# AE-HYU/monte_carlo_localization

Measured on AMD Instinct MI355X. Metric: MCL updates/sec (particle*beam/s), higher is better.
Workload: dtype f64; 1 GPU; 4194304 particles/GPU x 1081 beams, Spielberg_map (2000x2000 @ 0.05796), initial cloud N((0.0, 0.0, 0.0),(0.5 m,0.5 m,0.4 rad)) (tracking regime), action (0.05, 0.0, 0.01), stock sensor/motion params, multinomial resampling, Philox seed 42; the timed updates follow 5 warm-up updates (the particle set has resampled to motion-noise width); particles_total=4194304, beams=1081, parallelism=single GPU

## Files before the change

### include/mcl_hip_engine.h

```cpp
#ifndef MCL_HIP_ENGINE_H
#define MCL_HIP_ENGINE_H

#include <stddef.h>
#include <stdint.h>

#ifdef __cplusplus
extern "C" {
#endif

#define MCL_ABI_VERSION 1

typedef struct mcl_engine mcl_engine_t;

typedef enum {
    MCL_OK = 0,
    MCL_ERR_INVALID_ARG = -1,
    MCL_ERR_NOT_READY = -2,
    MCL_ERR_HIP = -3,
    MCL_ERR_NO_DEVICE = -4,
    MCL_ERR_UNSUPPORTED = -5,
    MCL_ERR_PEER = -6,
    MCL_ERR_TIMEOUT = -7
} mcl_status;

// ... 320 lines not shown
int mcl_host_skip_field(const int8_t *data, uint32_t width, uint32_t height, uint8_t *out, size_t n);
int mcl_host_skip_field_dir(const int8_t *data, uint32_t width, uint32_t height, int32_t quadrant, uint8_t *out, size_t n);
#define MCL_WEDGES 16
int mcl_host_skip_field_wedge(const int8_t *data, uint32_t width, uint32_t height, int32_t wedge, uint8_t *out, size_t n);
int mcl_host_skip_field_wedge_tight(const int8_t *data, uint32_t width, uint32_t height, int32_t wedge, uint8_t *out, size_t n);
int mcl_host_wedge_tight_table(int32_t wedge, int32_t *values, uint8_t *reachable, size_t n);
int mcl_host_sweep_global_layout(uint32_t width, uint32_t height, int32_t max_range_px, int64_t out[6]);
int mcl_get_wedge_fields(mcl_engine_t *h, uint8_t *out, size_t n, int32_t dims[3]);
int mcl_get_ring_fields(mcl_engine_t *h, uint8_t *out, size_t n);
int mcl_get_sweep_table(mcl_engine_t *h, double *out, size_t n, int32_t dims[3]);
int mcl_host_sort_key(const int32_t bbox[7], const int32_t *tilemap, int32_t ntx_abs, uint32_t width, uint32_t height,
                      const double *px, const double *py, const double *theta, int64_t n, int64_t n_layout, int32_t fine, uint32_t *keys);
int mcl_get_sort_order(mcl_engine_t *h, uint32_t *keys, uint32_t *perm, size_t n, int32_t bbox[7], int32_t *tilemap, size_t n_tiles,
                       int64_t *n_out, int32_t *fine);
int mcl_get_sort_record_form(mcl_engine_t *h, int32_t *heading_form);

typedef enum {
    MCL_BUF_X = 0, MCL_BUF_Y = 1, MCL_BUF_THETA = 2,
    MCL_BUF_QWEIGHT = 3,
    MCL_BUF_LOGW = 4,
    MCL_BUF_SCALARS = 5
} mcl_buffer_id;
int mcl_device_ptr(mcl_engine_t *h, int32_t which, void **dev_ptr);
int mcl_export_state(mcl_engine_t *h, double *d_x, double *d_y, double *d_theta, uint64_t *d_q);
int mcl_get_scalars(mcl_engine_t *h, double out[8]);
int mcl_get_host_scalars(const mcl_engine_t *h, double out[8]);
int mcl_stage_propagate(mcl_engine_t *h, const double *d_px, const double *d_py, const double *d_pth,
                        const uint64_t *d_cdf, int64_t n_parents, uint64_t q_total,
                        int64_t child_first, int64_t n_children_total,
                        const double action[3], const float *obs, int32_t n_beams);
// ... 74 lines not shown
```

### monte_carlo_localization_amd/csrc/mcl_engine.hip

```cpp
#include "../../include/mcl_hip_engine.h"

#include <hip/hip_runtime.h>
#include <hip/hip_ext.h>
#include <rocprim/device/device_radix_sort.hpp>

#include <algorithm>
#include <chrono>
#include <cmath>
#include <cstdio>
#include <cstring>
#include <string>
#include <vector>

#include "mcl_engine_internal.h"
#include "mcl_kernels.h"
#include "mcl_host_math.h"
#include "mcl_lfield.h"
#include "mcl_mount.h"

static_assert(MCL_WEDGES == mcl::kWedges || MCL_KWEDGES != 16, "include/mcl_hip_engine.h and csrc/mcl_wedge.h disagree");

using namespace mcl_host;

namespace {
// ... 66 lines not shown
    if (h->last_sweep_global == 2) {
        if (h->h_result[15] >= mcl::kFarWindowedMin / 2) { h->hyb_backoff = h->hyb_backoff ? std::min(32, 2 * h->hyb_backoff) : 1; h->hyb_skip = h->hyb_backoff; }
        else h->hyb_backoff = 0;
    }
    if (h->hyb_skip > 0) { --h->hyb_skip; return false; }
    return true;
}

int sweep_play(const mcl_engine *h, bool hybrid)
{
    if (hybrid) return mcl::kSwSide - (mcl::kSwHybReach + 2) - 3;
    if (h->sweep_global) return 1 << 20;
    return mcl::kSwSide - (h->P + 2) - 3;
}

int unit_play(const mcl_engine *h, int mode, bool hybrid)
{
    return h->env.no_bucket_cuts ? -1 : (mode_sweep(mode) ? sweep_play(h, hybrid) : 0);
}

int64_t max_sweep_units(int64_t n) { return (n + mcl::kSwUnit - 1) / mcl::kSwUnit + mcl::kSwMaxCuts + 2; }

int launch_sweep_plan(mcl_engine *h, int64_t n, int nwg, int g, bool hybrid)
{
    const int ngroups = mcl::kWedges / g;
    MCL_TRY(h->d_items.reserve(h, (size_t)max_sweep_units(n) * ngroups));
    MCL_TRY(h->d_centres.reserve(h, (size_t)max_sweep_units(n)));
    MCL_TRY(h->d_nitems.reserve(h, 1));
    const int play = sweep_play(h, hybrid);
    hipExtLaunchKernelGGL(mcl::k_sweep_plan, dim3(1), dim3(1024), mcl::kPlanLds, h->stream, nullptr, h->ev[EV_K0], 0, h->d_unit_sums.p, h->d_nunits.p, ngroups, nwg,
                          (double)(play / 2 - 1), h->env.sw_guide > 0 ? h->env.sw_guide : (h->sweep_global ? 3 : 2), h->d_items.p, h->d_centres.p, h->d_nitems.p);
    HIPCHK(h, hipGetLastError());
    return MCL_OK;
// ... 225 lines not shown

void ray_prep(mcl_engine *h, const RayPlan &p, const mcl::RayArgs &a)
{
    const dim3 grid((unsigned)((a.n + 255) / 256));
    if (!p.lists) {
        if (p.mode == MCL_RAYS_SKIP && !p.constants_ready)
            hipLaunchKernelGGL(mcl::k_particle_prep, grid, dim3(256), 0, h->stream, a.x, a.y, a.th, a.n, h->ox, h->oy, h->res, h->d_pc, h->d_angle, h->B,
                               (short4 *)nullptr, mcl::PrepClear{});
        return;
    }
    mcl::PrepClear clr{};
    clr.logw_acc = h->d_logw_acc; clr.far_flags = reinterpret_cast<uint32_t *>(h->d_far.p);
    clr.fix_count = h->d_fix_count; clr.fix_words = p.nseg * 8; clr.fix_over = h->d_fix_over; clr.exact_count = h->d_result + 14;
    if (p.sweep) clr.far_count = h->d_result + 15;
    if (p.ordered && !p.stale_layout) clr.bbox = h->d_bbox;
    clr.bbox_play = unit_play(h, p.mode, p.hyb);
    if (p.ordered && p.constants_ready) {
        clr.logw_acc = nullptr; clr.far_flags = nullptr;
        const mcl::PrepClear &pc0 = p.clear_passed;
        const bool done = p.clear_folded && clr.fix_count == pc0.fix_count && clr.fix_words == pc0.fix_words &&
                          clr.fix_over == pc0.fix_over && clr.exact_count == pc0.exact_count && clr.far_count == pc0.far_count &&
                          clr.bbox == pc0.bbox && clr.bbox_play == pc0.bbox_play && !clr.hist && !pc0.hist;
        if (!done) hipLaunchKernelGGL(mcl::k_prep_small, dim3(1), dim3(256), 0, h->stream, clr);
        if (!h->capturing) { h->prep_cache = clr; h->prep_cache_valid = true; h->prep_cache_n = a.n; }
    } else {
        hipLaunchKernelGGL(mcl::k_particle_prep, grid, dim3(256), 0, h->stream, a.x, a.y, a.th, a.n, h->ox, h->oy, h->res, h->d_pc, h->d_angle, h->B,
                           p.ordered ? (short4 *)nullptr : h->d_qr, clr);
    }
}

void ray_kernel_march(mcl_engine *h, const RayPlan &p, const mcl::RayArgs &a)
// ... 15 lines not shown
        hipLaunchKernelGGL(mcl::k_hist_partials, dim3(nparts), dim3(256), 0, h->stream, h->d_hist, h->d_histpart, h->d_tile_used);
        hipLaunchKernelGGL(mcl::k_hist_final, dim3(nparts), dim3(256), 0, h->stream, h->d_hist, h->d_histpart, h->d_tile_used);
        hipLaunchKernelGGL(mcl::k_sort_scatter, dim3(nb256), dim3(256), 0, h->stream, h->d_pc, a.th, n, h->d_skey, h->d_srank,
                           h->d_hist, h->d_pcs, h->d_ths, h->d_perm);
        return MCL_OK;
    }
    MCL_TRY(h->d_skey2.reserve(h, (size_t)h->cap));
    MCL_TRY(h->d_sval2.reserve(h, (size_t)h->cap));
    const int fine = sort_fine(h), key_bits = mcl::kSortKeyLog2 + mcl::sort_fine_bits(fine);
    size_t tb = 0;
    HIPCHK(h, rocprim::radix_sort_pairs(nullptr, tb, h->d_skey.p, h->d_skey2.p, h->d_srank.p, h->d_sval2.p, (size_t)n, 0, key_bits, h->stream));
    MCL_TRY(h->d_sort_tmp.reserve(h, tb));
    if (!(p.stale_layout && p.keys_written))
        hipLaunchKernelGGL(mcl::k_sort_keys, dim3(nb256), dim3(256), 0, h->stream, h->d_pc, a.th, n, h->Wp, h->Hp, h->d_bbox, h->d_skey, h->d_srank,
                           h->d_tilemap, ntx_abs, fine);
    tb = h->d_sort_tmp.cap;
    HIPCHK(h, rocprim::radix_sort_pairs(h->d_sort_tmp.p, tb, h->d_skey.p, h->d_skey2.p, h->d_srank.p, h->d_sval2.p, (size_t)n, 0, key_bits, h->stream));
    hipLaunchKernelGGL(mcl::k_sort_gather, dim3(nb256), dim3(256), 0, h->stream, h->d_pc, a.th, n, h->d_sval2, h->d_pcs, h->d_ths, h->d_perm,
                       p.sweep ? h->d_skey2 : (const uint32_t *)nullptr, h->d_bbox, h->d_cut_start, h->d_cut_end, fine, p.heading_form ? 1 : 0);
    h->order_last = {h->d_bbox.p, h->d_tilemap.p, n, fine, p.heading_form};
    return MCL_OK;
}

int ray_units(mcl_engine *h, const RayPlan &p, mcl::RayArgs &a)
{
    const int64_t n = a.n;
    const int nparts = (int)(mcl::kSortKeySpace / mcl::kHistTile);
    if (p.sweep) {
        const size_t mu = (size_t)max_sweep_units(n);
        MCL_TRY(h->d_unit_sums.reserve(h, mu * 2));
        MCL_TRY(h->d_unit_begin.reserve(h, mu + 1));
        MCL_TRY(h->d_nunits.reserve(h, 1));
        hipLaunchKernelGGL(mcl::k_unit_table, dim3(1), dim3(1024), 0, h->stream, h->d_bbox, n, h->d_hist, h->d_histpart, h->d_tile_used,
                           p.radix ? h->d_cut_start : (uint32_t *)nullptr, h->d_cut_end, h->d_unit_begin, h->d_nunits, (int)mu);
        hipLaunchKernelGGL(mcl::k_unit_sums, dim3((unsigned)std::min<int64_t>(max_sweep_units(n), (n + mcl::kSwUnit - 1) / mcl::kSwUnit + 256)), dim3(256), 0, h->stream, h->d_pcs, h->d_unit_begin, h->d_nunits,
                           h->d_unit_sums, p.radix ? (uint32_t *)nullptr : h->d_hist, h->d_tile_used, nparts);
    } else {
        if (!p.radix) hipLaunchKernelGGL(mcl::k_hist_clear, dim3(nparts), dim3(256), 0, h->stream, h->d_hist, h->d_tile_used);
        MCL_TRY(h->d_slice_mean.reserve(h, (size_t)p.nsl));
        hipLaunchKernelGGL(mcl::k_slice_means, dim3((unsigned)p.nsl), dim3(256), 0, h->stream, h->d_pcs, n, (n + p.nsl - 1) / p.nsl, h->d_slice_mean);
    }
    a.pcs = h->d_pcs; a.ths = h->d_ths; a.perm = h->d_perm; a.slice_mean = h->d_slice_mean;
    a.distw = h->d_distw; a.distw_stride = (size_t)h->Hp * h->Wps;
    return MCL_OK;
}

int ray_sweep_items(mcl_engine *h, const RayPlan &p, mcl::RayArgs &a)
{
    if (!h->d_Ltd) return fail(h, MCL_ERR_HIP, "k_rays_sweep: table not allocated (internal)");
    if (!h->ltd_ready) build_ltd(h);
    MCL_TRY(launch_sweep_plan(h, a.n, p.nseg, p.sweep_g, p.hyb));
// ... 450 lines not shown
const char *mcl_last_error(const mcl_engine_t *h) { return h ? h->err.c_str() : g_create_error.c_str(); }

static EnvKnobs read_knobs()
{
    EnvKnobs k;
    if (const char *e = getenv("MCL_CELL_MIN")) k.cell_min = atoll(e);
    if (const char *e = getenv("MCL_CELL_SLICE")) k.cell_slice = atoll(e);
    if (const char *e = getenv("MCL_QSLICES_PER_CU")) k.qslices_per_cu = atoi(e);
    if (const char *e = getenv("MCL_QSIDE")) k.qside = atoi(e);
    if (const char *e = getenv("MCL_SWEEP_G")) k.sweep_g = atoi(e);
    if (const char *e = getenv("MCL_TINY_POLL")) k.tiny_poll = atoi(e);
    if (const char *e = getenv("MCL_NO_COMPACT")) k.no_compact = atoi(e);
    if (const char *e = getenv("MCL_SORT")) k.sort_radix = std::strcmp(e, "radix") == 0 ? 1 : (std::strcmp(e, "hist") == 0 ? 0 : -1);
    if (const char *e = getenv("MCL_SORT_FINE")) k.sort_fine = atoi(e);
    if (const char *e = getenv("MCL_SORT_FINE_SUB")) k.sort_fine_sub = atoi(e);
    if (const char *e = getenv("MCL_FIX_WG")) k.fix_wg = atoi(e);
    if (const char *e = getenv("MCL_FIX_DEAL")) k.fix_deal_seg = std::strcmp(e, "seg") == 0;
    if (const char *e = getenv("MCL_DEBUG_WG")) k.debug_wg = e;
    k.no_bucket_cuts = getenv("MCL_NO_BUCKET_CUTS") != nullptr;
    if (const char *e = getenv("MCL_SWEEP_GLOBAL")) k.sweep_global = atoi(e) != 0;
    if (const char *e = getenv("MCL_SWEEP_HYBRID")) k.sweep_hybrid = atoi(e);
    if (const char *e = getenv("MCL_SW_GUIDE")) k.sw_guide = atoi(e);
    if (const char *e = getenv("MCL_SW_SPLIT16")) k.sw_split16 = atoi(e) != 0;
    if (const char *e = getenv("MCL_SWEEP_PAIRS")) k.sweep_pairs = atoi(e) != 0 ? 1 : 0;
    k.no_obs_overlap = getenv("MCL_NO_OBS_OVERLAP") != nullptr;
    k.no_prep_fold = getenv("MCL_NO_PREP_FOLD") != nullptr;
    k.no_stale_layout = getenv("MCL_NO_STALE_LAYOUT") != nullptr;
    k.comm_no_pregather = getenv("MCL_COMM_NO_PREGATHER") != nullptr;
    k.comm_no_lists = getenv("MCL_COMM_NO_LISTS") != nullptr;
    return k;
// ... 658 lines not shown
}

static int layout_mark(mcl_engine *h, int64_t n)
{
    h->layout.wanted = false;
    if (!mode_orders(choose_ray_mode(h, n, false)) || h->env.no_stale_layout) return MCL_OK;
    HIPCHK(h, hipEventRecord(h->layout.ev_children, h->stream));
    h->layout.wanted = true;
    return MCL_OK;
}

static int next_layout_launch(mcl_engine *h, int64_t n)
{
    if (!h->layout.wanted) return MCL_OK;
    h->layout.wanted = false;
    const int play = unit_play(h, choose_ray_mode(h, n, false), sweep_hybrid(h));
    HIPCHK(h, hipStreamWaitEvent(h->stream2, h->layout.ev_children, 0));
    hipLaunchKernelGGL(mcl::k_bbox_init, dim3(1), dim3(64), 0, h->stream2, h->layout.d_bbox_nx, play);
    launch_layout(h, h->stream2, n, h->layout.d_bbox_nx, h->layout.d_tilemark_nx, h->layout.d_tilemap_nx);
    HIPCHK(h, hipGetLastError());
    HIPCHK(h, hipEventRecord(h->layout.ev_layout, h->stream2));
    h->layout.pending = true;
    return MCL_OK;
}

int mcl_host::layout_adopt(mcl_engine *h, int64_t n)
{
    if (!h->layout.pending) return MCL_OK;
    HIPCHK(h, hipEventSynchronize(h->layout.ev_layout));
    std::swap(h->d_bbox, h->layout.d_bbox_nx); std::swap(h->d_tilemap, h->layout.d_tilemap_nx);
    h->layout.valid = true; h->layout.n = n; h->layout.pending = false;
// ... 841 lines not shown
        HIPCHK(h, hipMemcpyAsync(tilemap, o.tilemap, n_tiles * sizeof(int32_t), hipMemcpyDeviceToHost, h->stream));
    }
    HIPCHK(h, hipStreamSynchronize(h->stream));
    return MCL_OK;
}

int mcl_get_sort_record_form(mcl_engine_t *h, int32_t *heading_form)
{
    if (!h || !heading_form) return MCL_ERR_INVALID_ARG;
    const OrderLast &o = h->order_last;
    if (!o.bbox || o.n <= 0) return fail(h, MCL_ERR_NOT_READY, "the last ray stage did not order its particles through the radix sort");
    *heading_form = o.heading ? 1 : 0;
    return MCL_OK;
}

int mcl_get_ring_fields(mcl_engine_t *h, uint8_t *out, size_t n)
{
    if (!h || !out) return MCL_ERR_INVALID_ARG;
    if (!h->have_map || !h->d_distg) return fail(h, MCL_ERR_NOT_READY, "no map is set or the engine holds no ringed copies of the wedge fields");
    if (n != h->distg_stride * (size_t)mcl::kWedges) return fail(h, MCL_ERR_INVALID_ARG, "the ringed fields have the bytes of mcl_host_sweep_global_layout's allocation");
    HIPCHK(h, hipSetDevice(h->cfg.device));
    HIPCHK(h, hipMemcpyAsync(out, h->d_distg, n, hipMemcpyDeviceToHost, h->stream));
    HIPCHK(h, hipStreamSynchronize(h->stream));
    return MCL_OK;
}

int mcl_get_sweep_table(mcl_engine_t *h, double *out, size_t n, int32_t dims[3])
{
    if (!h) return MCL_ERR_INVALID_ARG;
    if (!h->have_map || h->B <= 0 || !h->d_Ltd || !h->ltd_ready)
// ... 632 lines not shown
```

### monte_carlo_localization_amd/csrc/mcl_engine_internal.h

```cpp
#pragma once
#include "../../include/mcl_hip_engine.h"

#include <hip/hip_runtime.h>
#include <hip/hip_ext.h>

#include <cstdint>
#include <string>
#include <vector>

#include "mcl_types.h"
#include "mcl_host_math.h"
#include "mcl_buffers.h"

enum { EV_START = 0, EV_RESAMPLE, EV_QUERY, EV_RAYS, EV_SENSOR, EV_K0, EV_K1, EV_COUNT };


constexpr unsigned long long kExactCap = 1ull << 16;
constexpr int kResultWords = 18;
constexpr int kResultStage = 40;
constexpr int kResultStamp = 32;

struct mcl_comm;
void comm_free(struct mcl_comm *c);
void comm_forget(struct mcl_comm *c);
// ... 18 lines not shown
    bool rays_bound = false;
    bool query_skipped = false;
};
struct NextLayout {
    bool wanted = false, pending = false, valid = false; int64_t n = 0;
    hipEvent_t ev_children = nullptr, ev_layout = nullptr;
    DevBuf<int> d_bbox_nx, d_tilemap_nx, d_tilemark_nx;
};
struct EnvKnobs {
    int64_t cell_min = 0, cell_slice = 0;
    int qslices_per_cu = 0, qside = 0, sweep_g = 0;
    int tiny_poll = 1, no_compact = 0;
    int sort_radix = -1;
    int sort_fine = -1;
    int sort_fine_sub = -1;
    int fix_wg = 0;
    bool fix_deal_seg = false;
    std::string debug_wg;
    bool no_bucket_cuts = false;
    bool sweep_global = false;
    int sweep_hybrid = 1;
    int sw_guide = 0;
    int sw_split16 = -1;
    int sweep_pairs = -1;
    bool no_obs_overlap = false;
    bool no_prep_fold = false;
    bool no_stale_layout = false;
    bool comm_no_pregather = false;
    bool comm_no_lists = false;
};
// ... 79 lines not shown
    unsigned long long list_epoch = 0;
    DevBuf<uint64_t> d_gcdf, d_gtop;
    DevBuf<double4> d_pcs;
    DevBuf<double> d_ths;
    DevBuf<uint32_t> d_perm, d_skey, d_srank;
    DevBuf<uint32_t> d_skey2, d_sval2;
    DevBuf<uint8_t> d_sort_tmp;
    DevBuf<uint32_t> d_tile_used;
    DevBuf<uint32_t> d_hist, d_histpart;
    DevBuf<int> d_bbox;
    OrderLast order_last;
    DevBuf<uint32_t> d_cut_start, d_cut_end;
    DevBuf<int> d_tilemap, d_tilemark;
    DevBuf<double2> d_slice_mean;
    DevBuf<double4> d_unit_sums;
    DevBuf<uint32_t> d_unit_begin;
    DevBuf<int> d_nunits;
    DevBuf<double4> d_pc;
    DevBuf<short4> d_qr;
    DevBuf<uint8_t> d_steps;
    DevBuf<unsigned long long> d_fix_list, d_fix_count;
    unsigned long long *d_fix_over = nullptr;
    DevBuf<unsigned long long> d_exact_list;
    unsigned long long fix_cap = 0; int fix_segments = 0;
    DevBuf<uint8_t> d_far;
    DevBuf<uint32_t> d_far_list;
    DevBuf<uint32_t> d_far_sorted, d_far_cnt;
    DevBuf<int4> d_items;
    DevBuf<int4> d_centres;
    DevBuf<int> d_nitems;
// ... 157 lines not shown
```

### monte_carlo_localization_amd/csrc/mcl_kernels.h

```cpp
#pragma once
#include "mcl_types.h"
#include <type_traits>
#include "mcl_ray_core.h"
#include "mcl_device_math.h"
#include "mcl_wedge.h"
#include "mcl_motion.h"
#include "mcl_sort_key.h"

namespace mcl {

constexpr int kRedBlocks = 1024;
constexpr int kRedThreads = 256;
__device__ __forceinline__ void final_sums_of(const double *__restrict__ part, int nb, double *__restrict__ scalars, double (*sm)[7]);


__device__ __forceinline__ uint64_t wave_incl_scan_u64(uint64_t v, int lane)
{
#pragma unroll
    for (int o = 1; o < 64; o <<= 1) {
        uint64_t t = (uint64_t)__shfl_up((long long)v, o, 64);
        if (lane >= o) v += t;
    }
    return v;
}
// ... 1311 lines not shown
__global__ __launch_bounds__(256) void k_sort_keys(const double4 *__restrict__ pc, const double *__restrict__ th, int64_t n, int Wp, int Hp,
                                                  const int *__restrict__ bbox, uint32_t *__restrict__ key_out, uint32_t *__restrict__ val_out,
                                                  const int *__restrict__ tilemap, int ntx_abs, int fine)
{
    const int64_t i = (int64_t)blockIdx.x * blockDim.x + threadIdx.x;
    if (i >= n) return;
    const double4 c = pc[i];
    key_out[i] = sort_key(bbox, tilemap, ntx_abs, cell_of(c.z * kSortSub, Wp * kSortSub - 1), cell_of(c.w * kSortSub, Hp * kSortSub - 1), th[i], n,
                          c.z * kSortSub - floor(c.z * kSortSub), c.w * kSortSub - floor(c.w * kSortSub), fine);
    val_out[i] = (uint32_t)i;
}
__global__ __launch_bounds__(256) void k_sort_gather(const double4 *__restrict__ pc, const double *__restrict__ th, int64_t n,
                                                    const uint32_t *__restrict__ order, double4 *__restrict__ pcs, double *__restrict__ ths,
                                                    uint32_t *__restrict__ perm, const uint32_t *__restrict__ sorted_keys = nullptr,
                                                    const int *__restrict__ bbox = nullptr, uint32_t *__restrict__ cut_start = nullptr,
                                                    uint32_t *__restrict__ cut_end = nullptr, int fine = 0, int heading_form = 0)
{
    const int64_t s = (int64_t)blockIdx.x * blockDim.x + threadIdx.x;
    if (s >= n) return;
    const uint32_t i = order[s];
    const double4 rec = pc[i];
    if (heading_form) { pcs[s] = particle_constants_of(rec); ths[s] = rec.x; }
    else { pcs[s] = rec; ths[s] = th[i]; }
    perm[s] = i;
    if (sorted_keys) {
        const SortLayout L = sort_layout(bbox, n, fine);
        if (L.cuts()) {
            const int sh = L.cut_shift();
            const uint32_t g = sorted_keys[s] >> sh;
            const uint32_t gp = s > 0 ? sorted_keys[s - 1] >> sh : 0xFFFFFFFFu;
            if (g != gp && g < (uint32_t)kSwMaxCuts) {
                cut_start[g] = (uint32_t)s + 1u;
                if (s > 0 && gp < (uint32_t)kSwMaxCuts) cut_end[gp] = (uint32_t)s;
            }
            if (s == n - 1 && g < (uint32_t)kSwMaxCuts) cut_end[g] = (uint32_t)n;
        }
    }
}

__global__ __launch_bounds__(256) void k_hist_clear(uint32_t *__restrict__ hist, uint32_t *__restrict__ tile_used)
{
    if (!tile_used[blockIdx.x]) return;
    const uint4 z = make_uint4(0u, 0u, 0u, 0u);
    for (int x = 0; x < kSortXcds; ++x) {
        uint4 *p = reinterpret_cast<uint4 *>(hist + (size_t)x * kSortKeySpace + (size_t)blockIdx.x * kHistTile) + threadIdx.x * 4;
#pragma unroll
        for (int k = 0; k < 4; ++k) p[k] = z;
    }
    __syncthreads();
    if (threadIdx.x == 0) tile_used[blockIdx.x] = 0u;
}
// ... 708 lines not shown
```

### monte_carlo_localization_amd/csrc/mcl_rays_sweep.h

```cpp
#pragma once

namespace mcl {

constexpr int kSwUnder = 127;
constexpr int kSwUnit = 1024;
constexpr int kSwFx = 32;
constexpr int kSwSide = 256;
#ifndef MCL_SW_PITCH
#define MCL_SW_PITCH 260
#endif
constexpr int kSwPitch = MCL_SW_PITCH;
static_assert(kSwPitch >= kSwSide && (kSwPitch % 4) == 0, "window rows are written as dwords");
constexpr int kSwWinBytes = kSwSide * kSwPitch;
#ifndef MCL_SW_HYB_PLAY
#define MCL_SW_HYB_PLAY 40
#endif
constexpr int kSwHybPlay = MCL_SW_HYB_PLAY;
constexpr int kSwHybReach = kSwSide - (kSwHybPlay + 3) - 2;
#if MCL_KWEDGES == 8
__device__ constexpr double kSwHybInvDx[2] = {1.0, 1.414213562373095};
__device__ constexpr double kSwHybInvDy[2] = {1.4142135623730951, 1.0};
#elif MCL_KWEDGES == 16
__device__ constexpr double kSwHybInvDx[4] = {1.0, 1.082392200292394, 1.414213562373095, 2.6131259297527527};
__device__ constexpr double kSwHybInvDy[4] = {2.613125929752753, 1.4142135623730951, 1.082392200292394, 1.0};
// ... 111 lines not shown
        }
        if (threadIdx.x == 1023) carry_sh = at + nu;
        __syncthreads();
        if (threadIdx.x == 0) nbig_sh = 0u;
        __syncthreads();
    }
    if (threadIdx.x == 0) {
        int M = (int)carry_sh;
        if (M > max_units) M = max_units;
        ub[M] = (uint32_t)n;
        m_out[0] = M;
    }
}

__global__ __launch_bounds__(256) void k_unit_sums(const double4 *__restrict__ pcs, const uint32_t *__restrict__ ub, const int *__restrict__ m_ptr,
                                                  double4 *__restrict__ out, uint32_t *__restrict__ hist, uint32_t *__restrict__ tile_used, int nparts)
{
    __shared__ double sm[4][7];
    if (hist) {
        for (int t = (int)blockIdx.x; t < nparts; t += (int)gridDim.x) {
            if (!tile_used[t]) continue;
            const uint4 z = make_uint4(0u, 0u, 0u, 0u);
            for (int x = 0; x < kSortXcds; ++x) {
                uint4 *p = reinterpret_cast<uint4 *>(hist + (size_t)x * kSortKeySpace + (size_t)t * kHistTile) + threadIdx.x * 4;
#pragma unroll
                for (int k = 0; k < 4; ++k) p[k] = z;
            }
            __syncthreads();
            if (threadIdx.x == 0) tile_used[t] = 0u;
        }
    }
    for (int u = (int)blockIdx.x; u < m_ptr[0]; u += (int)gridDim.x) {
    if (u != (int)blockIdx.x) __syncthreads();
// ... 857 lines not shown
```

### monte_carlo_localization_amd/csrc/mcl_sort_key.h

```cpp
#pragma once

#include <hip/hip_runtime.h>

#include <cmath>
#include <cstdint>

namespace mcl {

#ifndef MCL_SORT_SUB
#define MCL_SORT_SUB 1
#endif
constexpr int kSortSub = MCL_SORT_SUB;

#ifndef MCL_SORT_KEY_LOG2
#define MCL_SORT_KEY_LOG2 22
#endif
constexpr int kSortKeyLog2 = MCL_SORT_KEY_LOG2;
constexpr uint32_t kSortKeySpace = 1u << kSortKeyLog2;
#ifndef MCL_SORT_MAX_SUB
#define MCL_SORT_MAX_SUB 1
#endif
constexpr int kSortMaxFine = 10;
static_assert(kSortKeyLog2 + kSortMaxFine <= 32, "a key is one 32-bit word");
#ifndef MCL_SORT_FINE_DEFAULT
// ... 4 lines not shown
#endif
constexpr int kSortFineDefault = MCL_SORT_FINE_DEFAULT;
constexpr int kSortFineSubDefault = MCL_SORT_FINE_SUB_DEFAULT;

__host__ __device__ __forceinline__ int cell_of(double g, int hi)
{
    int c = (g > -1.0) ? ((g < 1e9) ? (int)floor(g) + 1 : hi) : 0;
    return c < 0 ? 0 : (c > hi ? hi : c);
}

#ifndef MCL_SORT_SUB_GATE
#define MCL_SORT_SUB_GATE 32.0
#endif
constexpr double kSortSubGate = MCL_SORT_SUB_GATE;
constexpr int kSortMaxSub = MCL_SORT_MAX_SUB;
struct SortLayout {
    int cs, tb, inner, ss;
    int fine;
    int fsub;
    uint32_t ntx;
    int tx0, ty0;
    bool compact;
    bool nocut;
    bool sparse;
    uint64_t ntiles;
    __host__ __device__ __forceinline__ int fine_sub() const { return fsub; }
    __host__ __device__ __forceinline__ int fine_heading() const { return fine - 2 * fine_sub(); }
    __host__ __device__ __forceinline__ int tile_shift() const { return 2 * inner + 2 * ss + tb + fine; }
    __host__ __device__ __forceinline__ int cut_shift() const { return sparse ? 2 * ss + tb + fine : tile_shift(); }
    __host__ __device__ __forceinline__ uint64_t cut_groups() const { return sparse ? ntiles << (2 * inner) : ntiles; }
    __host__ __device__ __forceinline__ bool cuts() const;
};
__host__ __device__ __forceinline__ int sort_fine_code(int fine, int fs = -1) { return (fine & 15) | (fs >= 0 ? (fs + 1) << 4 : 0); }
__host__ __device__ __forceinline__ int sort_fine_bits(int code) { const int f = code & 15; return f > kSortMaxFine ? kSortMaxFine : f; }
constexpr int kSwMaxCuts = 65536;
__host__ __device__ __forceinline__ bool SortLayout::cuts() const
{
    return compact && !nocut && cut_groups() <= (uint64_t)kSwMaxCuts && (cut_groups() << (cut_shift() - fine)) <= kSortKeySpace;
}
__host__ __device__ __forceinline__ SortLayout sort_layout(const int *__restrict__ bbox, int64_t n, int fine = 0)
{
    SortLayout L;
    L.fine = fine < 0 ? 0 : sort_fine_bits(fine);
    L.fsub = L.fine > 2 ? (L.fine - 2) / 4 : 0;
    if (fine > 0 && (fine >> 4) > 0) { L.fsub = (fine >> 4) - 1; if (2 * L.fsub > L.fine) L.fsub = L.fine / 2; }
    L.tx0 = bbox[0] >> 5; L.ty0 = bbox[1] >> 5;
    L.ntx = (uint32_t)((bbox[2] >> 5) - L.tx0 + 1);
    const uint32_t nty = (uint32_t)((bbox[3] >> 5) - L.ty0 + 1);
    L.compact = bbox[5] != 0;
    L.ntiles = L.compact ? (uint64_t)bbox[4] + 1u : (uint64_t)L.ntx * nty;
    double cells_est = (double)(bbox[2] - bbox[0] + 1) * (double)(bbox[3] - bbox[1] + 1);
    if (L.compact && (double)bbox[4] * 1024.0 < cells_est) cells_est = (double)bbox[4] * 1024.0;
    int cs = 0, tb = 6;
    L.nocut = bbox[6] < 0;
    L.sparse = cells_est > 0.0 && (double)n < 8.0 * cells_est;
    if (L.sparse) {
        cs = 5;
        const int play = bbox[6];
        while (play > 0 && cs > 1 && (1 << cs) >= play - 2 && (double)n * (double)(1 << (2 * cs - 2)) >= 128.0 * cells_est) --cs;
    }
    while (cs < 5 && ((L.ntiles << (10 - 2 * cs + tb)) > kSortKeySpace)) ++cs;
    while (tb > 0 && ((L.ntiles << (10 - 2 * cs + tb)) > kSortKeySpace)) --tb;
    const int inner = 5 - cs;
    const uint64_t ncell = L.ntiles << (2 * inner);
    while (tb < 8 && (ncell << (tb + 1)) <= kSortKeySpace) ++tb;
    int ss = 0;
    if (cs == 0 && tb == 8) {
        double per_bucket = cells_est > 0.0 ? (double)n / cells_est / 32.0 : 0.0;
        while (ss < kSortMaxSub && (ncell << (tb + 2 * (ss + 1))) <= kSortKeySpace && per_bucket >= kSortSubGate) { ++ss; per_bucket *= 0.25; }
    }
    L.cs = cs; L.tb = tb; L.inner = inner; L.ss = ss;
    return L;
}

__host__ __device__ __forceinline__ uint32_t sort_key(const int *__restrict__ bbox, const int *__restrict__ tilemap, int ntx_abs, int cx, int cy, double th,
                                                  int64_t n, double fx = 0.0, double fy = 0.0, int fine = 0)
{
    const bool in_box = cx >= bbox[0] && cx <= bbox[2] && cy >= bbox[1] && cy <= bbox[3];
    cx = cx < bbox[0] ? bbox[0] : (cx > bbox[2] ? bbox[2] : cx);
    cy = cy < bbox[1] ? bbox[1] : (cy > bbox[3] ? bbox[3] : cy);
    const SortLayout L = sort_layout(bbox, n, fine);
    const int cs = L.cs, tb = L.tb, inner = L.inner, ss = L.ss;
    uint32_t tile = (uint32_t)((cy >> 5) - L.ty0) * L.ntx + (uint32_t)((cx >> 5) - L.tx0);
    if (L.compact) tile = (uint32_t)tilemap[(cy >> 5) * ntx_abs + (cx >> 5)];
    const uint32_t ix = (uint32_t)(cx & 31) >> cs, iy = (uint32_t)(cy & 31) >> cs;
    uint64_t key = ((((uint64_t)tile << inner) | iy) << inner) | ix;
    if (ss > 0) {
        const uint32_t sx = (fx >= 0.0 && fx < 1.0) ? (uint32_t)(fx * (double)(1 << ss)) : 0u;
        const uint32_t sy = (fy >= 0.0 && fy < 1.0) ? (uint32_t)(fy * (double)(1 << ss)) : 0u;
        key = (((key << ss) | sy) << ss) | sx;
    }
    double f = th * 0.15915494309189533577;
    f -= floor(f);
    uint32_t tq = (f >= 0.0 && f < 1.0) ? (uint32_t)(f * (double)(1u << tb)) : 0u;
    if (tq >> tb) tq = (1u << tb) - 1u;
    key = (key << tb) | tq;
    const uint32_t coarse = key < kSortKeySpace ? (uint32_t)key : kSortKeySpace - 1u;
    if (L.fine == 0) return coarse;
    const int fs = L.fine_sub(), ft = L.fine_heading();
    uint32_t low = 0u;
    if (in_box && key < kSortKeySpace && fx >= 0.0 && fx < 1.0 && fy >= 0.0 && fy < 1.0 && f >= 0.0 && f < 1.0 && fabs(th) < 4294967296.0) {
// ... 10 lines not shown
```

### monte_carlo_localization_amd/engine.py

```python
from __future__ import annotations

import ctypes as C
import os

import numpy as np

_HERE = os.path.dirname(os.path.abspath(__file__))
LIB_PATH = os.environ.get("MCL_LIB") or os.path.join(_HERE, "libmcl_hip_engine.so")

MCL_OK = 0
MCL_ERR_INVALID_ARG = -1
MCL_ERR_NOT_READY = -2
MCL_ERR_PEER = -6
MCL_ERR_TIMEOUT = -7
RESAMPLE_MULTINOMIAL, RESAMPLE_SYSTEMATIC = 0, 1
WEIGHT_LOG, WEIGHT_PRODUCT = 0, 1
RAYS_AUTO, RAYS_MARCH, RAYS_SKIP, RAYS_QUAD, RAYS_CELL, RAYS_SWEEP = 0, 1, 2, 3, 4, 5
BUF_X, BUF_Y, BUF_THETA, BUF_QWEIGHT, BUF_LOGW, BUF_SCALARS = range(6)

EXPORTS = [
    "mcl_abi_version", "mcl_default_config", "mcl_create", "mcl_destroy", "mcl_last_error", "mcl_set_map",
    "mcl_get_max_range_px", "mcl_get_sensor_table", "mcl_set_beam_angles", "mcl_set_particles",
    "mcl_get_particles", "mcl_get_weights", "mcl_sample_particles", "mcl_particle_mean", "mcl_update",
    "mcl_sensor_update", "mcl_expected_pose", "mcl_get_stage_timings", "mcl_get_resample_indices",
    "mcl_get_ray_steps", "mcl_get_log_weights", "mcl_get_counters", "mcl_get_ray_kernel_ms", "mcl_device_ptr",
    "mcl_stage_propagate", "mcl_stage_weights", "mcl_stage_finish", "mcl_scan_weights", "mcl_export_state",
    "mcl_get_scalars", "mcl_host_sensor_table", "mcl_host_skip_field", "mcl_init_particles_pose", "mcl_init_global",
    "mcl_update_scan", "mcl_get_ray_kernel_id", "mcl_host_skip_field_dir", "mcl_host_skip_field_wedge", "mcl_export_records", "mcl_get_effective_sample_size", "mcl_get_host_scalars", "mcl_stage_resample_records", "mcl_stage_resample", "mcl_stage_rays",
    "mcl_set_reserved_cus", "mcl_stage_resample_indices", "mcl_stage_motion_records", "mcl_stage_distinct_parents", "mcl_export_records_at",
    "mcl_group_create", "mcl_group_destroy", "mcl_group_last_error", "mcl_group_size", "mcl_group_engine", "mcl_group_set_map",
    "mcl_group_set_beam_angles", "mcl_group_set_particles", "mcl_group_init_particles_pose", "mcl_group_init_global",
    "mcl_group_update", "mcl_group_expected_pose", "mcl_group_get_particles", "mcl_group_get_weights",
    "mcl_group_get_resample_indices", "mcl_group_get_stage_timings", "mcl_group_exchange_bytes",
    "mcl_set_debug_count_probes", "mcl_set_debug_force_exact", "mcl_set_particles_shard", "mcl_get_compact_list", "mcl_compact_chunk_bytes", "mcl_export_compact",
    "mcl_stage_resample_compact", "mcl_group_exchanged_lists", "mcl_get_ray_steps16", "mcl_get_planned_ray_kernel",
    "mcl_stream_wait_external", "mcl_external_wait_stream", "mcl_export_compact_async", "mcl_stage_resample_compact_async",
    "mcl_stage_rays_async", "mcl_stage_weights_async", "mcl_stage_complete", "mcl_stage_keep",
    "mcl_comm_available", "mcl_comm_unique_id", "mcl_comm_create", "mcl_comm_destroy", "mcl_comm_update", "mcl_comm_stats", "mcl_comm_set_lists", "mcl_comm_get_vector", "mcl_comm_last_exchange", "mcl_comm_selftest",
    "mcl_host_sweep_global_layout", "mcl_get_ray_kernel_variant", "mcl_host_skip_field_wedge_tight", "mcl_host_wedge_tight_table",
    "mcl_get_wedge_fields", "mcl_get_ring_fields", "mcl_get_sweep_table", "mcl_host_sort_key", "mcl_get_sort_order", "mcl_get_sort_record_form",
    "mcl_default_kld_config", "mcl_set_kld", "mcl_get_particle_count", "mcl_get_kld_state", "mcl_host_kld_bins", "mcl_host_kld_target",
    "mcl_default_cluster_config", "mcl_pose_clusters", "mcl_get_cluster_labels",
    "mcl_query_scans", "mcl_score_poses", "mcl_get_query_counters",
    "mcl_default_search_config", "mcl_global_search", "mcl_get_search_scores", "mcl_get_search_bytes", "mcl_host_search_lattice",
    "mcl_host_search_headings", "mcl_init_particles_mixture",
    "mcl_global_search_sequence", "mcl_host_search_sequence_offsets", "mcl_host_relative_poses",
    "mcl_default_search_stream_config", "mcl_global_search_streamed", "mcl_host_search_slabs",
    "mcl_global_search_beam", "mcl_host_search_beam_grid", "mcl_get_search_beam_table",
    "mcl_default_search_prune_config", "mcl_global_search_pruned", "mcl_get_search_bounds", "mcl_host_search_blocks", "mcl_host_lf_pool",
    "mcl_host_search_bound_table", "mcl_host_search_prune_next", "mcl_global_search_sequence_pruned",
    "mcl_default_refine_config", "mcl_refine_poses", "mcl_refine_poses_beam", "mcl_get_refine_scores", "mcl_get_refine_bytes", "mcl_host_refine_window",
    "mcl_host_refine_reduce", "mcl_refine_poses_sequence", "mcl_host_refine_sequence_offsets",
    "mcl_default_recovery_config", "mcl_set_recovery", "mcl_get_recovery_state", "mcl_set_recovery_state", "mcl_host_recovery_step",
    "mcl_set_recovery_proposal", "mcl_get_recovery_proposal", "mcl_host_recovery_proposal",
    "mcl_default_likelihood_field_config", "mcl_set_likelihood_field", "mcl_get_likelihood_field", "mcl_get_likelihood_table",
# ... 813 lines not shown
        raise EngineError(f"mcl_host_sweep_global_layout rc={rc}", rc)
    return dict(ok=bool(out[0]), pitch=int(out[1]), rows=int(out[2]), stride=int(out[3]), alloc=int(out[4]), max_offset=int(out[5]))


def host_skip_field_wedge_tight(grid, wedge: int) -> np.ndarray:
    g = _c(grid, np.int8)
    H, W = g.shape
    out = np.empty((H + 1, W + 1), np.uint8)
    rc = load_library().mcl_host_skip_field_wedge_tight(_p(g), C.c_uint32(W), C.c_uint32(H), C.c_int32(wedge), _p(out), C.c_size_t(out.size))
    if rc != MCL_OK:
        raise EngineError(f"mcl_host_skip_field_wedge_tight rc={rc}")
    return out


SORT_KEY_LOG2, SORT_MAX_FINE = 22, 10


def sort_fine_code(fine: int, fine_sub: int | None = None) -> int:
    if not 0 <= int(fine) <= SORT_MAX_FINE or (fine_sub is not None and not 0 <= 2 * int(fine_sub) <= int(fine)):
        raise EngineError(f"sort key: fine={fine} fine_sub={fine_sub} (0 .. {SORT_MAX_FINE} bits, at most half of them per axis)", MCL_ERR_INVALID_ARG)
    return int(fine) | ((int(fine_sub) + 1) << 4 if fine_sub is not None else 0)


def sort_tile_grid(width: int, height: int):
    return (int(width) >> 5) + 1, (int(height) >> 5) + 1


def host_sort_key(bbox, tilemap, width: int, height: int, px, py, theta, fine: int = 0, n_layout: int | None = None,
                  fine_sub: int | None = None) -> np.ndarray:
    bb = _c(np.asarray(bbox).reshape(-1)[:7], np.int32)
# ... 394 lines not shown
        return out, int(dims[2])

    def sort_order(self):
        n, fine = C.c_int64(), C.c_int32()
        self._chk(self.lib.mcl_get_sort_order(self._h, None, None, C.c_size_t(0), None, None, C.c_size_t(0), C.byref(n), C.byref(fine)),
                  "mcl_get_sort_order")
        keys, perm, bbox = np.empty(n.value, np.uint32), np.empty(n.value, np.uint32), np.empty(7, np.int32)
        H, W = self.map_shape
        ntx, nty = sort_tile_grid(W, H)
        tm = np.empty(ntx * nty, np.int32) if ntx * nty <= 8192 else None
        self._chk(self.lib.mcl_get_sort_order(self._h, _p(keys), _p(perm), C.c_size_t(n.value), _p(bbox), _p(tm) if tm is not None else None,
                                              C.c_size_t(tm.size if tm is not None else 0), None, None), "mcl_get_sort_order")
        return dict(keys=keys, perm=perm, bbox=bbox, tilemap=tm, n=int(n.value), fine=int(fine.value) & 15,
                    fine_sub=(int(fine.value) >> 4) - 1 if int(fine.value) >> 4 else None)

    def sort_record_form(self) -> str:
        f = C.c_int32()
        self._chk(self.lib.mcl_get_sort_record_form(self._h, C.byref(f)), "mcl_get_sort_record_form")
        return "heading" if f.value else "full"

    def particle_count(self) -> int:
        n = C.c_int64()
        self._chk(self.lib.mcl_get_particle_count(self._h, C.byref(n)), "mcl_get_particle_count")
        return n.value

    def pose_clusters(self, max_clusters=16, **cfg_fields):
        cfg = default_cluster_config(**cfg_fields)
        out = np.zeros(int(max_clusters), CLUSTER_DTYPE)
        n = C.c_int64()
        tot = (C.c_uint64 * 3)()
# ... 607 lines not shown
```

Measured before the change: 934.8 billion particle*beam/s.

## Add bounding-box sort key layout and fuse unit sums into sort gather

Adds a 'box' sort layout in which the radix sort key is the row-major cell index within the particle bounding box, with optional sub-cell bits, in place of the tile-map indexing. It is on by default when radix sort and sweep mode apply. The sort gather kernel now also writes per-block partial sums and bounding boxes, which k_unit_sums then combines in place of re-reading every sorted particle. This is meant to tighten spatial locality for the sweep ray kernel and cut a pass over the particles. The cost is that bucket cuts are disabled under box mode, and a debug accessor for unit stats is added.

Measured after the change: 934.4 billion particle*beam/s. No clear change (-0.0%).

```diff
diff --git a/include/mcl_hip_engine.h b/include/mcl_hip_engine.h
--- a/include/mcl_hip_engine.h
+++ b/include/mcl_hip_engine.h
@@ -358,6 +358,7 @@
 int mcl_get_sort_order(mcl_engine_t *h, uint32_t *keys, uint32_t *perm, size_t n, int32_t bbox[7], int32_t *tilemap, size_t n_tiles,
                        int64_t *n_out, int32_t *fine);
 int mcl_get_sort_record_form(mcl_engine_t *h, int32_t *heading_form);
+int mcl_get_unit_stats(mcl_engine_t *h, double *stats, uint32_t *begin, size_t n_units, int64_t *n_units_out);
 
 typedef enum {
     MCL_BUF_X = 0, MCL_BUF_Y = 1, MCL_BUF_THETA = 2,
diff --git a/monte_carlo_localization_amd/csrc/mcl_engine.hip b/monte_carlo_localization_amd/csrc/mcl_engine.hip
--- a/monte_carlo_localization_amd/csrc/mcl_engine.hip
+++ b/monte_carlo_localization_amd/csrc/mcl_engine.hip
@@ -104,9 +104,12 @@
     return mcl::kSwSide - (h->P + 2) - 3;
 }
 
-int unit_play(const mcl_engine *h, int mode, bool hybrid)
-{
-    return h->env.no_bucket_cuts ? -1 : (mode_sweep(mode) ? sweep_play(h, hybrid) : 0);
+bool sort_radix(const mcl_engine *h, int64_t n);
+int unit_play(const mcl_engine *h, int mode, bool hybrid, int64_t n)
+{
+    if (h->env.no_bucket_cuts) return -1;
+    const int play = mode_sweep(mode) ? sweep_play(h, hybrid) : 0;
+    return play > 0 && h->env.sort_box && sort_radix(h, n) ? (play | mcl::kSortBoxBit) : play;
 }
 
 int64_t max_sweep_units(int64_t n) { return (n + mcl::kSwUnit - 1) / mcl::kSwUnit + mcl::kSwMaxCuts + 2; }
@@ -362,7 +365,7 @@
     clr.fix_count = h->d_fix_count; clr.fix_words = p.nseg * 8; clr.fix_over = h->d_fix_over; clr.exact_count = h->d_result + 14;
     if (p.sweep) clr.far_count = h->d_result + 15;
     if (p.ordered && !p.stale_layout) clr.bbox = h->d_bbox;
-    clr.bbox_play = unit_play(h, p.mode, p.hyb);
+    clr.bbox_play = unit_play(h, p.mode, p.hyb, a.n);
     if (p.ordered && p.constants_ready) {
         clr.logw_acc = nullptr; clr.far_flags = nullptr;
         const mcl::PrepClear &pc0 = p.clear_passed;
@@ -408,10 +411,12 @@
     if (!(p.stale_layout && p.keys_written))
         hipLaunchKernelGGL(mcl::k_sort_keys, dim3(nb256), dim3(256), 0, h->stream, h->d_pc, a.th, n, h->Wp, h->Hp, h->d_bbox, h->d_skey, h->d_srank,
                            h->d_tilemap, ntx_abs, fine);
+    if (p.sweep) MCL_TRY(h->d_unit_parts.reserve(h, std::max((size_t)nb256, ((size_t)h->cap + 255) / 256) * 2));
     tb = h->d_sort_tmp.cap;
     HIPCHK(h, rocprim::radix_sort_pairs(h->d_sort_tmp.p, tb, h->d_skey.p, h->d_skey2.p, h->d_srank.p, h->d_sval2.p, (size_t)n, 0, key_bits, h->stream));
     hipLaunchKernelGGL(mcl::k_sort_gather, dim3(nb256), dim3(256), 0, h->stream, h->d_pc, a.th, n, h->d_sval2, h->d_pcs, h->d_ths, h->d_perm,
-                       p.sweep ? h->d_skey2 : (const uint32_t *)nullptr, h->d_bbox, h->d_cut_start, h->d_cut_end, fine, p.heading_form ? 1 : 0);
+                       p.sweep ? h->d_skey2 : (const uint32_t *)nullptr, h->d_bbox, h->d_cut_start, h->d_cut_end, fine, p.heading_form ? 1 : 0,
+                       p.sweep ? h->d_unit_parts.p : (double4 *)nullptr);
     h->order_last = {h->d_bbox.p, h->d_tilemap.p, n, fine, p.heading_form};
     return MCL_OK;
 }
@@ -428,7 +433,8 @@
         hipLaunchKernelGGL(mcl::k_unit_table, dim3(1), dim3(1024), 0, h->stream, h->d_bbox, n, h->d_hist, h->d_histpart, h->d_tile_used,
                            p.radix ? h->d_cut_start : (uint32_t *)nullptr, h->d_cut_end, h->d_unit_begin, h->d_nunits, (int)mu);
         hipLaunchKernelGGL(mcl::k_unit_sums, dim3((unsigned)std::min<int64_t>(max_sweep_units(n), (n + mcl::kSwUnit - 1) / mcl::kSwUnit + 256)), dim3(256), 0, h->stream, h->d_pcs, h->d_unit_begin, h->d_nunits,
-                           h->d_unit_sums, p.radix ? (uint32_t *)nullptr : h->d_hist, h->d_tile_used, nparts);
+                           h->d_unit_sums, p.radix ? (uint32_t *)nullptr : h->d_hist, h->d_tile_used, nparts,
+                           p.radix ? h->d_unit_parts.p : (const double4 *)nullptr, h->d_bbox, n);
     } else {
         if (!p.radix) hipLaunchKernelGGL(mcl::k_hist_clear, dim3(nparts), dim3(256), 0, h->stream, h->d_hist, h->d_tile_used);
         MCL_TRY(h->d_slice_mean.reserve(h, (size_t)p.nsl));
@@ -909,6 +915,7 @@
     if (const char *e = getenv("MCL_SORT")) k.sort_radix = std::strcmp(e, "radix") == 0 ? 1 : (std::strcmp(e, "hist") == 0 ? 0 : -1);
     if (const char *e = getenv("MCL_SORT_FINE")) k.sort_fine = atoi(e);
     if (const char *e = getenv("MCL_SORT_FINE_SUB")) k.sort_fine_sub = atoi(e);
+    if (const char *e = getenv("MCL_SORT_BOX")) k.sort_box = atoi(e) != 0;
     if (const char *e = getenv("MCL_FIX_WG")) k.fix_wg = atoi(e);
     if (const char *e = getenv("MCL_FIX_DEAL")) k.fix_deal_seg = std::strcmp(e, "seg") == 0;
     if (const char *e = getenv("MCL_DEBUG_WG")) k.debug_wg = e;
@@ -1597,7 +1604,7 @@
 {
     if (!h->layout.wanted) return MCL_OK;
     h->layout.wanted = false;
-    const int play = unit_play(h, choose_ray_mode(h, n, false), sweep_hybrid(h));
+    const int play = unit_play(h, choose_ray_mode(h, n, false), sweep_hybrid(h), n);
     HIPCHK(h, hipStreamWaitEvent(h->stream2, h->layout.ev_children, 0));
     hipLaunchKernelGGL(mcl::k_bbox_init, dim3(1), dim3(64), 0, h->stream2, h->layout.d_bbox_nx, play);
     launch_layout(h, h->stream2, n, h->layout.d_bbox_nx, h->layout.d_tilemark_nx, h->layout.d_tilemap_nx);
@@ -2469,6 +2476,24 @@
     return MCL_OK;
 }
 
+int mcl_get_unit_stats(mcl_engine_t *h, double *stats, uint32_t *begin, size_t n_units, int64_t *n_units_out)
+{
+    if (!h) return MCL_ERR_INVALID_ARG;
+    if (!h->d_nunits || !h->d_unit_sums || !h->d_unit_begin) return fail(h, MCL_ERR_NOT_READY, "no ray stage of this engine has made k_rays_sweep's units");
+    HIPCHK(h, hipSetDevice(h->cfg.device));
+    int m = 0;
+    HIPCHK(h, hipMemcpyAsync(&m, h->d_nunits, sizeof(int), hipMemcpyDeviceToHost, h->stream));
+    HIPCHK(h, hipStreamSynchronize(h->stream));
+    if (m < 0 || (size_t)m * 2 > h->d_unit_sums.cap || (size_t)m + 1 > h->d_unit_begin.cap) return fail(h, MCL_ERR_NOT_READY, "the unit count on the device is not one the unit buffers hold");
+    if (n_units_out) *n_units_out = m;
+    if (!stats && !begin) return MCL_OK;
+    if (n_units != (size_t)m) return fail(h, MCL_ERR_INVALID_ARG, "stats has 8 doubles and begin one word per unit of the last ray stage (begin one more)");
+    if (stats) HIPCHK(h, hipMemcpyAsync(stats, h->d_unit_sums, (size_t)m * 2 * sizeof(double4), hipMemcpyDeviceToHost, h->stream));
+    if (begin) HIPCHK(h, hipMemcpyAsync(begin, h->d_unit_begin, ((size_t)m + 1) * sizeof(uint32_t), hipMemcpyDeviceToHost, h->stream));
+    HIPCHK(h, hipStreamSynchronize(h->stream));
+    return MCL_OK;
+}
+
 int mcl_get_ring_fields(mcl_engine_t *h, uint8_t *out, size_t n)
 {
     if (!h || !out) return MCL_ERR_INVALID_ARG;
diff --git a/monte_carlo_localization_amd/csrc/mcl_engine_internal.h b/monte_carlo_localization_amd/csrc/mcl_engine_internal.h
--- a/monte_carlo_localization_amd/csrc/mcl_engine_internal.h
+++ b/monte_carlo_localization_amd/csrc/mcl_engine_internal.h
@@ -56,6 +56,7 @@
     int sort_radix = -1;
     int sort_fine = -1;
     int sort_fine_sub = -1;
+    bool sort_box = true;
     int fix_wg = 0;
     bool fix_deal_seg = false;
     std::string debug_wg;
@@ -165,6 +166,7 @@
     DevBuf<int> d_tilemap, d_tilemark;
     DevBuf<double2> d_slice_mean;
     DevBuf<double4> d_unit_sums;
+    DevBuf<double4> d_unit_parts;
     DevBuf<uint32_t> d_unit_begin;
     DevBuf<int> d_nunits;
     DevBuf<double4> d_pc;
diff --git a/monte_carlo_localization_amd/csrc/mcl_kernels.h b/monte_carlo_localization_amd/csrc/mcl_kernels.h
--- a/monte_carlo_localization_amd/csrc/mcl_kernels.h
+++ b/monte_carlo_localization_amd/csrc/mcl_kernels.h
@@ -1349,18 +1349,25 @@
                                                     const uint32_t *__restrict__ order, double4 *__restrict__ pcs, double *__restrict__ ths,
                                                     uint32_t *__restrict__ perm, const uint32_t *__restrict__ sorted_keys = nullptr,
                                                     const int *__restrict__ bbox = nullptr, uint32_t *__restrict__ cut_start = nullptr,
-                                                    uint32_t *__restrict__ cut_end = nullptr, int fine = 0, int heading_form = 0)
+                                                    uint32_t *__restrict__ cut_end = nullptr, int fine = 0, int heading_form = 0,
+                                                    double4 *__restrict__ parts = nullptr)
 {
     const int64_t s = (int64_t)blockIdx.x * blockDim.x + threadIdx.x;
-    if (s >= n) return;
-    const uint32_t i = order[s];
-    const double4 rec = pc[i];
-    if (heading_form) { pcs[s] = particle_constants_of(rec); ths[s] = rec.x; }
-    else { pcs[s] = rec; ths[s] = th[i]; }
-    perm[s] = i;
+    if (s >= n && !parts) return;
+    bool cut = false;
+    double px = NAN, py = NAN;
+    if (s < n) {
+        const uint32_t i = order[s];
+        const double4 rec = pc[i];
+        if (heading_form) { pcs[s] = particle_constants_of(rec); ths[s] = rec.x; }
+        else { pcs[s] = rec; ths[s] = th[i]; }
+        perm[s] = i;
+        px = rec.z; py = rec.w;
+    }
     if (sorted_keys) {
         const SortLayout L = sort_layout(bbox, n, fine);
-        if (L.cuts()) {
+        cut = L.cuts();
+        if (cut && s < n) {
             const int sh = L.cut_shift();
             const uint32_t g = sorted_keys[s] >> sh;
             const uint32_t gp = s > 0 ? sorted_keys[s - 1] >> sh : 0xFFFFFFFFu;
@@ -1370,6 +1377,22 @@
             }
             if (s == n - 1 && g < (uint32_t)kSwMaxCuts) cut_end[g] = (uint32_t)n;
         }
+    }
+    if (!parts || !sorted_keys || cut) return;
+    const bool ok = px == px && py == py && fabs(px) < 1e9 && fabs(py) < 1e9;
+    double sx = ok ? px : 0.0, sy = ok ? py : 0.0, cnt = ok ? 1.0 : 0.0;
+    double x0 = ok ? px : INFINITY, x1 = ok ? px : -INFINITY, y0 = ok ? py : INFINITY, y1 = ok ? py : -INFINITY;
+    sx = wave_sum(sx); sy = wave_sum(sy); cnt = wave_sum(cnt);
+    x0 = -wave_max(-x0); x1 = wave_max(x1); y0 = -wave_max(-y0); y1 = wave_max(y1);
+    __shared__ double sm[4][7];
+    const int w = threadIdx.x >> 6;
+    if ((threadIdx.x & 63) == 0) { sm[w][0] = sx; sm[w][1] = sy; sm[w][2] = cnt; sm[w][3] = x0; sm[w][4] = x1; sm[w][5] = y0; sm[w][6] = y1; }
+    __syncthreads();
+    if (threadIdx.x == 0) {
+        parts[2 * (size_t)blockIdx.x] = make_double4(sm[0][0] + sm[1][0] + sm[2][0] + sm[3][0], sm[0][1] + sm[1][1] + sm[2][1] + sm[3][1],
+                                                     sm[0][2] + sm[1][2] + sm[2][2] + sm[3][2], 0.0);
+        parts[2 * (size_t)blockIdx.x + 1] = make_double4(fmin(fmin(sm[0][3], sm[1][3]), fmin(sm[2][3], sm[3][3])), fmax(fmax(sm[0][4], sm[1][4]), fmax(sm[2][4], sm[3][4])),
+                                                         fmin(fmin(sm[0][5], sm[1][5]), fmin(sm[2][5], sm[3][5])), fmax(fmax(sm[0][6], sm[1][6]), fmax(sm[2][6], sm[3][6])));
     }
 }
 
diff --git a/monte_carlo_localization_amd/csrc/mcl_rays_sweep.h b/monte_carlo_localization_amd/csrc/mcl_rays_sweep.h
--- a/monte_carlo_localization_amd/csrc/mcl_rays_sweep.h
+++ b/monte_carlo_localization_amd/csrc/mcl_rays_sweep.h
@@ -149,9 +149,26 @@
 }
 
 __global__ __launch_bounds__(256) void k_unit_sums(const double4 *__restrict__ pcs, const uint32_t *__restrict__ ub, const int *__restrict__ m_ptr,
-                                                  double4 *__restrict__ out, uint32_t *__restrict__ hist, uint32_t *__restrict__ tile_used, int nparts)
+                                                  double4 *__restrict__ out, uint32_t *__restrict__ hist, uint32_t *__restrict__ tile_used, int nparts,
+                                                  const double4 *__restrict__ parts = nullptr, const int *__restrict__ bbox = nullptr, int64_t n = 0)
 {
     __shared__ double sm[4][7];
+    if (parts && !sort_layout(bbox, n).cuts()) {
+        constexpr int kPer = kSwUnit / 256;
+        const int64_t nb = (n + 255) / 256;
+        const int M = m_ptr[0];
+        for (int64_t u = (int64_t)blockIdx.x * blockDim.x + threadIdx.x; u < M; u += (int64_t)gridDim.x * blockDim.x) {
+            double4 a = make_double4(0.0, 0.0, 0.0, 0.0), b = make_double4(INFINITY, -INFINITY, INFINITY, -INFINITY);
+            for (int k = 0; k < kPer && u * kPer + k < nb; ++k) {
+                const double4 pa = parts[2 * (size_t)(u * kPer + k)], pb = parts[2 * (size_t)(u * kPer + k) + 1];
+                a.x += pa.x; a.y += pa.y; a.z += pa.z;
+                b.x = fmin(b.x, pb.x); b.y = fmax(b.y, pb.y); b.z = fmin(b.z, pb.z); b.w = fmax(b.w, pb.w);
+            }
+            out[2 * (size_t)u] = a;
+            out[2 * (size_t)u + 1] = b;
+        }
+        return;
+    }
     if (hist) {
         for (int t = (int)blockIdx.x; t < nparts; t += (int)gridDim.x) {
             if (!tile_used[t]) continue;
diff --git a/monte_carlo_localization_amd/csrc/mcl_sort_key.h b/monte_carlo_localization_amd/csrc/mcl_sort_key.h
--- a/monte_carlo_localization_amd/csrc/mcl_sort_key.h
+++ b/monte_carlo_localization_amd/csrc/mcl_sort_key.h
@@ -42,6 +42,14 @@
 #endif
 constexpr double kSortSubGate = MCL_SORT_SUB_GATE;
 constexpr int kSortMaxSub = MCL_SORT_MAX_SUB;
+#ifndef MCL_SORT_MAX_SUB_BOX
+#define MCL_SORT_MAX_SUB_BOX 3
+#endif
+constexpr int kSortMaxSubBox = MCL_SORT_MAX_SUB_BOX;
+constexpr int kSortBoxBit = 1 << 30;
+constexpr uint64_t kSortBoxCells = 1u << (kSortKeyLog2 - 10);
+__host__ __device__ __forceinline__ int sort_play(int word) { return word < 0 ? word : (word & ~kSortBoxBit); }
+__host__ __device__ __forceinline__ bool sort_box_asked(int word) { return word > 0 && (word & kSortBoxBit) != 0; }
 struct SortLayout {
     int cs, tb, inner, ss;
     int fine;
@@ -51,12 +59,14 @@
     bool compact;
     bool nocut;
     bool sparse;
+    bool box;
+    uint32_t bw;
     uint64_t ntiles;
     __host__ __device__ __forceinline__ int fine_sub() const { return fsub; }
     __host__ __device__ __forceinline__ int fine_heading() const { return fine - 2 * fine_sub(); }
     __host__ __device__ __forceinline__ int tile_shift() const { return 2 * inner + 2 * ss + tb + fine; }
     __host__ __device__ __forceinline__ int cut_shift() const { return sparse ? 2 * ss + tb + fine : tile_shift(); }
-    __host__ __device__ __forceinline__ uint64_t cut_groups() const { return sparse ? ntiles << (2 * inner) : ntiles; }
+    __host__ __device__ __forceinline__ uint64_t cut_groups() const { return box ? 1u : (sparse ? ntiles << (2 * inner) : ntiles); }
     __host__ __device__ __forceinline__ bool cuts() const;
 };
 __host__ __device__ __forceinline__ int sort_fine_code(int fine, int fs = -1) { return (fine & 15) | (fs >= 0 ? (fs + 1) << 4 : 0); }
@@ -64,7 +74,7 @@
 constexpr int kSwMaxCuts = 65536;
 __host__ __device__ __forceinline__ bool SortLayout::cuts() const
 {
-    return compact && !nocut && cut_groups() <= (uint64_t)kSwMaxCuts && (cut_groups() << (cut_shift() - fine)) <= kSortKeySpace;
+    return !box && compact && !nocut && cut_groups() <= (uint64_t)kSwMaxCuts && (cut_groups() << (cut_shift() - fine)) <= kSortKeySpace;
 }
 __host__ __device__ __forceinline__ SortLayout sort_layout(const int *__restrict__ bbox, int64_t n, int fine = 0)
 {
@@ -82,9 +92,23 @@
     int cs = 0, tb = 6;
     L.nocut = bbox[6] < 0;
     L.sparse = cells_est > 0.0 && (double)n < 8.0 * cells_est;
+    L.box = false; L.bw = 0u;
+    if (sort_box_asked(bbox[6]) && !L.sparse && bbox[2] >= bbox[0] && bbox[3] >= bbox[1]) {
+        const uint64_t bw = (uint64_t)((int64_t)bbox[2] - bbox[0] + 1), bh = (uint64_t)((int64_t)bbox[3] - bbox[1] + 1);
+        if (bw <= kSortBoxCells && bh <= kSortBoxCells && bw * bh <= kSortBoxCells) {
+            const uint64_t ncell = bw * bh;
+            const int tb = 8;
+            double per_bucket = cells_est > 0.0 ? (double)n / cells_est / 32.0 : 0.0;
+            int ss = 0;
+            while (ss < kSortMaxSubBox && (ncell << (tb + 2 * (ss + 1))) <= kSortKeySpace && per_bucket >= kSortSubGate) { ++ss; per_bucket *= 0.25; }
+            L.box = true; L.bw = (uint32_t)bw; L.ntiles = 1u;
+            L.cs = 0; L.tb = tb; L.inner = 0; L.ss = ss;
+            return L;
+        }
+    }
     if (L.sparse) {
         cs = 5;
-        const int play = bbox[6];
+        const int play = sort_play(bbox[6]);
         while (play > 0 && cs > 1 && (1 << cs) >= play - 2 && (double)n * (double)(1 << (2 * cs - 2)) >= 128.0 * cells_est) --cs;
     }
     while (cs < 5 && ((L.ntiles << (10 - 2 * cs + tb)) > kSortKeySpace)) ++cs;
@@ -110,9 +134,10 @@
     const SortLayout L = sort_layout(bbox, n, fine);
     const int cs = L.cs, tb = L.tb, inner = L.inner, ss = L.ss;
     uint32_t tile = (uint32_t)((cy >> 5) - L.ty0) * L.ntx + (uint32_t)((cx >> 5) - L.tx0);
-    if (L.compact) tile = (uint32_t)tilemap[(cy >> 5) * ntx_abs + (cx >> 5)];
+    if (L.compact && !L.box) tile = (uint32_t)tilemap[(cy >> 5) * ntx_abs + (cx >> 5)];
     const uint32_t ix = (uint32_t)(cx & 31) >> cs, iy = (uint32_t)(cy & 31) >> cs;
     uint64_t key = ((((uint64_t)tile << inner) | iy) << inner) | ix;
+    if (L.box) key = (uint64_t)(uint32_t)(cy - bbox[1]) * L.bw + (uint32_t)(cx - bbox[0]);
     if (ss > 0) {
         const uint32_t sx = (fx >= 0.0 && fx < 1.0) ? (uint32_t)(fx * (double)(1 << ss)) : 0u;
         const uint32_t sy = (fy >= 0.0 && fy < 1.0) ? (uint32_t)(fy * (double)(1 << ss)) : 0u;
diff --git a/monte_carlo_localization_amd/engine.py b/monte_carlo_localization_amd/engine.py
--- a/monte_carlo_localization_amd/engine.py
+++ b/monte_carlo_localization_amd/engine.py
@@ -38,7 +38,7 @@
     "mcl_stage_rays_async", "mcl_stage_weights_async", "mcl_stage_complete", "mcl_stage_keep",
     "mcl_comm_available", "mcl_comm_unique_id", "mcl_comm_create", "mcl_comm_destroy", "mcl_comm_update", "mcl_comm_stats", "mcl_comm_set_lists", "mcl_comm_get_vector", "mcl_comm_last_exchange", "mcl_comm_selftest",
     "mcl_host_sweep_global_layout", "mcl_get_ray_kernel_variant", "mcl_host_skip_field_wedge_tight", "mcl_host_wedge_tight_table",
-    "mcl_get_wedge_fields", "mcl_get_ring_fields", "mcl_get_sweep_table", "mcl_host_sort_key", "mcl_get_sort_order", "mcl_get_sort_record_form",
+    "mcl_get_wedge_fields", "mcl_get_ring_fields", "mcl_get_sweep_table", "mcl_host_sort_key", "mcl_get_sort_order", "mcl_get_sort_record_form", "mcl_get_unit_stats",
     "mcl_default_kld_config", "mcl_set_kld", "mcl_get_particle_count", "mcl_get_kld_state", "mcl_host_kld_bins", "mcl_host_kld_target",
     "mcl_default_cluster_config", "mcl_pose_clusters", "mcl_get_cluster_labels",
     "mcl_query_scans", "mcl_score_poses", "mcl_get_query_counters",
@@ -882,6 +882,7 @@
 
 
 SORT_KEY_LOG2, SORT_MAX_FINE = 22, 10
+SORT_BOX_BIT, SORT_BOX_CELLS, SORT_BOX_MAX_SUB = 1 << 30, 1 << 12, 3
 
 
 def sort_fine_code(fine: int, fine_sub: int | None = None) -> int:
@@ -1306,6 +1307,15 @@
         return dict(keys=keys, perm=perm, bbox=bbox, tilemap=tm, n=int(n.value), fine=int(fine.value) & 15,
                     fine_sub=(int(fine.value) >> 4) - 1 if int(fine.value) >> 4 else None)
 
+    def unit_stats(self):
+        fn = self.lib.mcl_get_unit_stats
+        fn.argtypes = [C.c_void_p, C.c_void_p, C.c_void_p, C.c_size_t, C.POINTER(C.c_int64)]
+        m = C.c_int64()
+        self._chk(fn(self._h, None, None, C.c_size_t(0), C.byref(m)), "mcl_get_unit_stats")
+        stats, begin = np.empty((m.value, 8), np.float64), np.empty(m.value + 1, np.uint32)
+        self._chk(fn(self._h, _p(stats), _p(begin), C.c_size_t(m.value), None), "mcl_get_unit_stats")
+        return dict(begin=begin, sums=stats[:, :3].copy(), boxes=stats[:, 4:].copy())
+
     def sort_record_form(self) -> str:
         f = C.c_int32()
         self._chk(self.lib.mcl_get_sort_record_form(self._h, C.byref(f)), "mcl_get_sort_record_form")
```
